# Ryo1011gd/ParticleMethod_FSI

Hardware: AMD Instinct MI355X
Metric: particle-steps/sec + achieved HBM GB/s, dam-break, 1/2/4/8 MI355X (higher is better)
Workload: dtype f64; 1 GPU; d1m: 3-D dam break (SURVEY 8d D1M, BASELINE configs[1]), 1397200 particles, ~1397200 per GPU; particles=1397200, dim=3, module=dam, parallelism=single

## Files before the change

include/mph_gpu.h:

```cpp
#ifndef MPH_GPU_H_INCLUDED
#define MPH_GPU_H_INCLUDED

#include <stddef.h>

#ifdef __cplusplus
extern "C" {
#endif

#define MPH_TYPE_COUNT 6
#define MPH_MAX_NEIGHBOR_COUNT 512
#define MPH_ABI_VERSION 6

typedef enum MphModule {
    MPH_MODULE_BAR = 0,
    MPH_MODULE_DAM = 1,
    MPH_MODULE_TUREK_HRON = 2,
    MPH_MODULE_ROLLING1 = 3,
    MPH_MODULE_HYDROELASTIC = 4,
    MPH_MODULE_NONE = 5
} MphModule;

typedef enum MphWallMotion {
    MPH_WALL_RIGID = 0,
    MPH_WALL_ROLLING = 1
// ... 229 lines not shown
    void* host_user;
    int n_glob;
    const int* ids;
    const double* cuts;
} MphSlabOptions;
int mph_create_slab(MphCtx** ctx, const MphConfig* cfg, int n, const int* property, const double* pos,
                    const double* pos0, const double* vel, int device, const MphSlabOptions* opt);
int mph_slab_window(const MphConfig* cfg, int rank, int nranks, int axis, const double* cuts, double* out2);
int mph_dist_selftest(int device);
int mph_dist_info(const MphCtx* ctx, int* out8);
int mph_dist_overlap(const MphCtx* ctx, double* out5);
int mph_list_stats(MphCtx* ctx, double* mean, int* max);
int mph_list_layout(MphCtx* ctx, long long out6[6]);
int mph_idle_wall_stats(MphCtx* ctx, long long out2[2]);
int mph_lean_step_stats(MphCtx* ctx, long long out2[2]);
int mph_neighbor_rows(MphCtx* ctx, int first, int count, int* counts, int* ids, long long ids_cap);
int mph_owned_count(const MphCtx* ctx);
int mph_owned_ids(MphCtx* ctx, int* out_ids);
int mph_slab_bounds(const MphConfig* cfg, int rank, int nranks, int axis, const double* cuts, double* out3);
int mph_slab_owner(const MphConfig* cfg, int nranks, int axis, const double* cuts, double c);

#ifdef __cplusplus
}
#endif
#endif
```

particlemethod_fsi_amd/csrc/mph_ctx.h:

```cpp
#pragma once

#include <hip/hip_runtime.h>

#include <map>
#include <string>
#include <thread>
#include <vector>

#include "mph_internal.h"
#include "mph_kernels.h"

struct MphDist;

struct MphCtx {
    int device = 0;
    int n = 0;
    int n_glob = 0;
    MphConfig cfg{};
    mph::HostDerived h{};
    mph::DevParams P{};
    mph::DevTables tables{};
    std::string err;
    std::thread out_thread;
    int out_rc = 0;
    double time = 0.0;
    bool stepped = false;
    hipStream_t stream = nullptr;
    hipGraphExec_t graph1 = nullptr, graph8 = nullptr;
    hipGraphExec_t graph1t = nullptr;
    bool batch_steps = false;
    int pending = 0;
    bool unchecked = false;
    void* hs_pin = nullptr;
    hipEvent_t ev_status = nullptr;
    bool phase_timing = false;
    std::vector<hipEvent_t> ev8, ev_vir;
    double phase_ms[3] = {0.0, 0.0, 0.0};
    std::vector<int> prop;
    std::vector<double> pos0;
    std::vector<int> gid;
    mph::StructureInit S;
    std::vector<int> sl_orig;
    std::vector<int> sl_s;
    int* order = nullptr;
// ... 119 lines not shown
    void join(hipStream_t waiting, hipStream_t from) override
    {
        hipEvent_t e = nullptr;
        (void)hipEventCreate(&e);
        (void)hipEventRecord(e, from);
        floors.push_back(e);
        pending[waiting] = (int)floors.size() - 1;
    }
    ~EventProfiler() override
    {
        for (auto& r : recs) { (void)hipEventDestroy(r.a); (void)hipEventDestroy(r.b); }
        for (auto e : floors) (void)hipEventDestroy(e);
    }
};

void enqueue_step(const Launch& L, bool last, hipEvent_t* ev = nullptr);

void ctx_set_global_error(const std::string& msg);
int ctx_create(MphCtx** out, const MphConfig* cfg, int n, const int* property, const double* pos,
               const double* pos0, const double* vel, int device, MphDist* dist, const int* ids = nullptr,
               int n_glob = 0);
template <typename T>
int fetch(MphCtx* c, const T* d, std::vector<T>& h, size_t count)
{
    h.resize(count);
    if (count) MPH_HIP_OK(c, hipMemcpyAsync(h.data(), d, sizeof(T) * count, hipMemcpyDeviceToHost, c->stream));
    return MPH_OK;
}

inline int glob_id(const MphCtx* c, int k) { return c->gid.empty() ? k : c->gid[k]; }

// ... 14 lines not shown
```

particlemethod_fsi_amd/csrc/mph_ctx.hip:

```cpp
#include <hip/hip_runtime.h>

#include <algorithm>
#include <cstring>
#include <string>

#include "mph_dist.h"
#include "mph_env.h"

using namespace mph;

namespace mph {

int ctx_fail(MphCtx* c, int code, const std::string& msg)
{
    if (c) c->err = msg;
    return code;
}

int ctx_hip_fail(MphCtx* c, hipError_t e, const char* what)
{
    return ctx_fail(c, e == hipErrorOutOfMemory ? MPH_ERR_DEVICE_OOM : MPH_ERR_HIP,
                    std::string(what) + ": " + hipGetErrorString(e));
}

// ... 42 lines not shown
    DevState hs;
    std::memcpy(&hs, c->hs_pin, kStateHead);
    return ctx_state_status(c, hs);
}

int ctx_status(MphCtx* c)
{
    MPH_CK(ctx_status_enqueue(c));
    MPH_HIP_OK(c, hipStreamSynchronize(c->stream));
    return ctx_status_landed(c);
}

int drop_graphs(MphCtx* c)
{
    MPH_HIP_OK(c, hipStreamSynchronize(c->stream));
    for (hipGraphExec_t* g : {&c->graph1, &c->graph1t, &c->graph8})
        if (*g) {
            MPH_HIP_OK(c, hipGraphExecDestroy(*g));
            *g = nullptr;
        }
    return MPH_OK;
}

int ctx_replay(MphCtx* c, int n)
{
    for (; n >= 8; n -= 8) MPH_HIP_OK(c, hipGraphLaunch(c->graph8, c->stream));
    for (; n > 1; --n) MPH_HIP_OK(c, hipGraphLaunch(c->graph1t ? c->graph1t : c->graph1, c->stream));
    if (n == 1) MPH_HIP_OK(c, hipGraphLaunch(c->graph1, c->stream));
    return MPH_OK;
}

void ctx_fill_launch(MphCtx* c)
{
    Launch& L = c->L;
    set_uniforms(c->P);
    if (env_int("MPH_LIST_FULL", 0) == 1) c->P.rlf = 3.0e38f;
    c->lazy_walls = !c->dist && env_int("MPH_LAZY_WALLS", 1) != 0;
    L.lean_ok = env_int("MPH_LEAN_STEPS", 1) != 0;
    L.lean_search = L.lean_ok && lean_search_ok(c->P);
    L.P = &c->P;
    L.stream = c->stream;
    L.xcd_bal_min = env_is("MPH_XCD_BAL_MIN", "") ? (1 << 20) : env_int("MPH_XCD_BAL_MIN", 1 << 20);
    L.S = &c->Sd;
}

}

extern "C" {

int mph_synchronize(MphCtx* c)
{
    if (!c) return MPH_ERR_ARG;
    MPH_CK(ctx_flush(c));
    MPH_HIP_OK(c, hipStreamSynchronize(c->stream));
// ... 11 lines not shown
    return MPH_OK;
}

void mph_destroy(MphCtx* c)
{
    if (!c) return;
    if (c->out_thread.joinable()) c->out_thread.join();
    (void)hipSetDevice(c->device);
    (void)ctx_flush(c);
    if (c->hs_pin) (void)hipHostFree(c->hs_pin);
    if (c->ev_status) (void)hipEventDestroy(c->ev_status);
    if (c->stream) (void)hipStreamSynchronize(c->stream);
    if (c->graph1) (void)hipGraphExecDestroy(c->graph1);
    if (c->graph1t) (void)hipGraphExecDestroy(c->graph1t);
    if (c->graph8) (void)hipGraphExecDestroy(c->graph8);
    for (auto* v : {&c->ev8, &c->ev_vir})
        for (hipEvent_t e : *v) (void)hipEventDestroy(e);
    if (c->dist) dist_free(c);
    for (void* p : c->allocs) (void)hipFree(p);
    if (c->stream) (void)hipStreamDestroy(c->stream);
    delete c;
}

}
```

particlemethod_fsi_amd/csrc/mph_device.h:

```cpp
#pragma once

#include <hip/hip_runtime.h>
#include <hip/hip_ext.h>

#include <climits>
#include <type_traits>

#include "mph_kernels.h"
#include "mph_params.h"

namespace mph {

__device__ __forceinline__ double mod_exact(double x, double w)
{
#pragma clang fp contract(off)
    return x - w * floor(x / w);
}

template <bool FAST>
__device__ __forceinline__ double image_exact(double d, double w, double hw, double w075)
{
#pragma clang fp contract(off)
    const double s = d + hw;
    double m;
// ... 113 lines not shown
{
    const int id = MAX ? INT_MIN : INT_MAX;
    auto op = [](int a, int b) { return MAX ? max(a, b) : min(a, b); };
    v = op(v, __builtin_amdgcn_update_dpp(id, v, 0x111, 0xf, 0xf, false));
    v = op(v, __builtin_amdgcn_update_dpp(id, v, 0x112, 0xf, 0xf, false));
    v = op(v, __builtin_amdgcn_update_dpp(id, v, 0x113, 0xf, 0xf, false));
    v = op(v, __builtin_amdgcn_update_dpp(id, v, 0x114, 0xf, 0xe, false));
    v = op(v, __builtin_amdgcn_update_dpp(id, v, 0x118, 0xf, 0xc, false));
    v = op(v, __builtin_amdgcn_update_dpp(id, v, 0x142, 0xa, 0xf, false));
    v = op(v, __builtin_amdgcn_update_dpp(id, v, 0x143, 0xc, 0xf, false));
    return __builtin_amdgcn_readlane(v, 63);
}

__device__ __forceinline__ int wave_min(int v) { return wave_reduce_dpp<false>(v); }
__device__ __forceinline__ int wave_max(int v) { return wave_reduce_dpp<true>(v); }

__device__ __forceinline__ void move_and_wrap(const DevParams& P, const DevState* st, Soa& B, int p,
                                              double& x, double& y, double& z)
{
#pragma clang fp contract(off)
    const int t = B.type[p];
    if (P.module == MPH_MODULE_TUREK_HRON && dev_is_fluid(t)) {
        const double ymin = 0.0, ymax = 0.41, umax = 1.0, h = ymax - ymin;
        if (x <= 0.01) {
            const double uy = y - ymin;
            B.vx[p] = (1.5 * 4.0 * umax / (h * h)) * uy * (h - uy);
            B.vy[p] = 0.0;
            B.vz[p] = 0.0;
        }
        if (x > 1.5 && st->time < 0.7) {
// ... 157 lines not shown
```

particlemethod_fsi_amd/csrc/mph_kernels.h:

```cpp
#pragma once

#include <hip/hip_runtime.h>

#include "mph_params.h"

namespace mph {

struct StructDev {
    int* orig = nullptr;
    int* slot_of = nullptr;
    int* bidx = nullptr;
    int n_own = 0;
    int n_inner = 0;
    int wo = 0, wi = 0;
    int* ocnt = nullptr;
    int* icnt = nullptr;
    int* eo_nb = nullptr;
    int* ei_nb = nullptr;
    double4* wx0 = nullptr;
    double* L = nullptr;
    double2* lame = nullptr;
    double* inv_rho = nullptr;
    int* clamp = nullptr;
    double4* x0 = nullptr;
// ... 41 lines not shown
    int width = 0;
    double probe_h = 0.0;
    long long* counters = nullptr;
    double* ring = nullptr;
    double* partial = nullptr;
    double* trk = nullptr;
    double* prb = nullptr;
    const int* track_sorted = nullptr;
    const int* track_map = nullptr;
    const double* probes = nullptr;
};

struct StepForm {
    bool lazy = false;
    bool lean_search = false, lean_pass_a = false;
};

struct Launch {
    const DevParams* P = nullptr;
    const DevTables* T = nullptr;
    DevState* st = nullptr;
    hipStream_t stream = nullptr;
    Profiler* prof = nullptr;
    Soa A, B;
    int* dst_of = nullptr;
    int *key = nullptr, *slot = nullptr, *tmp = nullptr, *cnt = nullptr, *start = nullptr, *bsum = nullptr;
    int *nbr = nullptr, *ncount = nullptr, *nbcount = nullptr;
    unsigned long long *lhdr = nullptr, *lgap = nullptr;
    int* wface = nullptr;
    VSrc vsrc;
    int xcd_bal_min = 1 << 20;
    unsigned char* cmap = nullptr;
    int cmap_bytes = 0;
    bool lean_ok = false, lean_search = false;
    StepForm form;
    double *pres = nullptr, *gx = nullptr, *gy = nullptr, *gz = nullptr, *pa = nullptr;
    double *dens_a = nullptr, *vstrain = nullptr, *divp = nullptr;
    double4 *fpart = nullptr;
    double4 *rec = nullptr;
    double4 *force = nullptr, *acc = nullptr;
    const StructDev* S = nullptr;
    const MonitorDev* mon = nullptr;
};

inline Launch trim_outputs(Launch L)
{
    L.dens_a = L.vstrain = L.divp = nullptr;
    if (!L.P->surface) L.gx = L.gy = L.gz = L.pa = nullptr;
    L.force = L.acc = nullptr;
    return L;
}

inline Launch step_launch(const Launch& L, bool last)
{
    Launch S = last ? L : trim_outputs(L);
    S.form.lazy = !last && L.cmap && !L.mon;
    S.form.lean_search = S.form.lazy && L.lean_ok && L.lean_search;
    S.form.lean_pass_a = S.form.lazy && L.lean_ok && !L.P->surface;
    return S;
}

struct SampleDev {
    double origin[3], spacing[3];
    int count[3];
    int tile[3];
    int tiles[3];
    int mask;
    double h;
};


int monitor_blocks(int n);
void launch_monitor(const Launch& L, const MonitorDev& M);
long long sample_tiling(SampleDev& G, int run_axis);
// ... 44 lines not shown
```

particlemethod_fsi_amd/csrc/mph_params.h:

```cpp
#pragma once
#include <cmath>

#include <cstddef>
#include <cstdint>

#include "../../include/mph_gpu.h"


namespace mph {

constexpr int kTypes = MPH_TYPE_COUNT;
constexpr int kMaxNeighbor = MPH_MAX_NEIGHBOR_COUNT;
constexpr int kTile = 64;
constexpr int kAlignRows = 128;
constexpr int kMaxJumps = 6;
#ifndef MPH_TILE_EXTRA
#define MPH_TILE_EXTRA kAlignRows
#endif
constexpr int kTileRows = kMaxNeighbor + MPH_TILE_EXTRA;
#ifndef MPH_TILE_PAD
#define MPH_TILE_PAD 1
#endif
constexpr int kTileStride = kTile * (kTileRows + MPH_TILE_PAD);
#if defined(__HIPCC__)
// ... 129 lines not shown
    int overflow;
    int pad0;
    int seam_occ[2];
    int seam_step;
    int seam_pad;
    int seg_work[kXcdSegs];
    int xcd_frac[9];
    int xcd_pad[3];
    unsigned long long lazy_steps;
    unsigned idle_waves[kXcdSegs];
    int seg_lwork[kXcdSegs];
    int seg_swork[kXcdSegs];
    int xcd_sfrac[9];
    int xcd_spad[3];
    unsigned long long lean_search_steps, lean_pass_a_steps;
};
constexpr size_t kStateHead = offsetof(DevState, seg_work);

#if defined(__HIPCC__)
#define MPH_HD __host__ __device__
#else
#define MPH_HD
#endif

MPH_HD inline int jump_count(unsigned long long hdr) { return (int)(hdr >> 56); }
MPH_HD inline int gap_begin(unsigned long long gap, int k) { return (int)((gap >> (8 * k)) & 0xff); }
MPH_HD inline int gap_end(unsigned long long hdr, int k) { return (int)((hdr >> (8 * k)) & 0xff); }

#ifndef MPH_PA_EQR
#define MPH_PA_EQR 1
// ... 74 lines not shown
```

particlemethod_fsi_amd/csrc/mph_passes.hip:

```cpp
#include <cstdio>
#include <cstdlib>
#include <type_traits>

#include "mph_list.h"

namespace mph {

__device__ __forceinline__ void own_velocity(const Soa& A, int i, double& vx, double& vy, double& vz)
{
    const double2 b = A.p6[3 * (size_t)i + 1], c = A.p6[3 * (size_t)i + 2];
    vx = b.y; vy = c.x; vz = c.y;
}


struct PassA {
    double da = 0.0, g0 = 0.0, g1 = 0.0, g2 = 0.0, vs = 0.0, dv = 0.0;
    double s0 = 0.0, s1 = 0.0, s2 = 0.0, v0 = 0.0, v1 = 0.0, v2 = 0.0;
};

template <bool FORCE, bool EQR = false, bool LEAN = false>
__device__ __forceinline__ void pass_a_term(const DevParams& P, const double* s_ratio, const double* s_mu, int ti,
                                            int tj, bool solid, double q0, double q1, double q2, double r2,
                                            double dvx, double dvy, double dvz, PassA& o)
{
// ... 313 lines not shown
        for (int u = 0; u < U; ++u) {
            const unsigned off = ok[u] ? (unsigned)jj[u] * 16u : kGatherOob;
            const double2 a = buf_ld16(recr, off), b = buf_ld16(recr, off == kGatherOob ? off : off + ps16);
            X[u] = a.x; Y[u] = a.y; Z[u] = b.x; PJ[u] = b.y;
        }
#pragma unroll
        for (int u = 0; u < U; ++u) {
            asm volatile("" ::"v"(X[u]), "v"(Y[u]), "v"(Z[u]), "v"(PJ[u]));
            if (!ok[u]) continue;
            pass_b_term<FAST, SURF, DIM>(P, s_ratio, gx, gy, gz, pa, jj[u], TT[u], X[u], Y[u], Z[u], PJ[u], ti,
                                         solid, xi, yi, zi, gxi, gyi, gzi, pai, ai, dscale, cpv, f0, f1, f2);
        }
    }
}

template <bool SURF, int DIM>
#ifndef MPH_PB_WPE
#define MPH_PB_WPE 0
#endif
#if MPH_PB_WPE
#define MPH_PB_ATTR __attribute__((amdgpu_waves_per_eu(MPH_PB_WPE)))
#else
#define MPH_PB_ATTR
#endif
__global__ __launch_bounds__(MPH_LB) MPH_PB_ATTR void k_pass_b(DevParams P, const DevTables* __restrict__ T, Soa A,
                                                const double4* __restrict__ rec,
                                                const double4* __restrict__ fpart,
                                                const double* __restrict__ gx,
                                                const double* __restrict__ gy,
                                                const double* __restrict__ gz,
                                                const double* __restrict__ pa,
                                                const int* __restrict__ nbr,
                                                const int* __restrict__ ncount,
                                                const unsigned long long* __restrict__ lhdr,
                                                const unsigned long long* __restrict__ lgap,
                                                double4* __restrict__ force, double4* __restrict__ acc,
                                                Soa B, int phase, int* __restrict__ wface, StructHook H,
                                                const DevState* __restrict__ st)
{
    const int n = dev_n(P);
    const int lb = list_block(st, n);
    if (lb < 0) return;
    __shared__ double s_ratio[kTypes * kTypes];
    if (SURF) {
        if (threadIdx.x < kTypes * kTypes) s_ratio[threadIdx.x] = T->ratio[threadIdx.x];
        __syncthreads();
    }
    const int i = lb * blockDim.x + threadIdx.x;
    const int ii = i < n ? i : n - 1;
    const double xi = A.x[ii], yi = A.y[ii], zi = A.z[ii];
    bool live = i < n;
    if (phase) {
        const int f = wface[__builtin_amdgcn_readfirstlane(i >> 6)];
        if (phase == 1 ? f != 0 : f == 0) return;
    }
    if (wave_all_ghosts(P, A, live, ii)) {
        if (live) B.id[i] = A.id[i];
        return;
    }
    if (live && P.slab_axis >= 0 && A.id[ii] < 0) {
        B.id[i] = A.id[i];
        live = false;
    }
    const bool fast = wave_search_interior(P, st, live, xi, yi, zi);
    if (!live) return;
    const int ti = A.type[ii];
    const bool solid = dev_is_struct(ti);
    const double4 fp = fpart[ii];
    double f0 = fp.x, f1 = fp.y, f2 = fp.z;
    double gxi = 0.0, gyi = 0.0, gzi = 0.0, pai = 0.0, ai = 0.0;
    if (SURF) {
        gxi = gx[ii]; gyi = gy[ii]; gzi = gz[ii]; pai = pa[ii];
        ai = T->cofa[ti] * P.cofk * P.cofk;
    }
    const int end = !force && dev_is_wall(ti) ? 0 : (ncount[i] < kTileRows ? ncount[i] : kTileRows);
    const unsigned long long hdr = wave_hdr(lhdr, i);
    const bool plain = (hdr >> 56) == 0;
    const RowMask M = row_mask(hdr, lgap, i, end);
    const NbrList NL = nbr_list(nbr, i);
    if (fast)
        pass_b_loop<true, SURF, DIM>(P, s_ratio, rec, gx, gy, gz, pa, NL, plain, M, end, ti, solid, xi, yi, zi, gxi,
                                     gyi, gzi, pai, ai, f0, f1, f2);
    else
        pass_b_loop<false, SURF, DIM>(P, s_ratio, rec, gx, gy, gz, pa, NL, plain, M, end, ti, solid, xi, yi, zi, gxi,
                                      gyi, gzi, pai, ai, f0, f1, f2);
    double vxi, vyi, vzi;
    own_velocity(A, i, vxi, vyi, vzi);
    double vo0 = vxi, vo1 = vyi, vo2 = vzi;
    double xo0 = xi, xo1 = yi, xo2 = zi;
    double4 ao = make_double4(0.0, 0.0, 0.0, 0.0);
    if (dev_is_fluid(ti) || solid) {
        const double m = T->mass[ti], im = T->inv_mass[ti];
        f0 += m * P.gravity[0];
        f1 += m * P.gravity[1];
        f2 += m * P.gravity[2];
        vo0 += f0 * im * P.dt;
        vo1 += f1 * im * P.dt;
        vo2 += f2 * im * P.dt;
        if (!solid) {
            ao = make_double4(f0 * im, f1 * im, f2 * im, 0.0);
            xo0 += vo0 * P.dt;
            xo1 += vo1 * P.dt;
            xo2 += vo2 * P.dt;
        }
    }
    if (force) {
        force[i] = make_double4(f0, f1, f2, 0.0);
        acc[i] = ao;
    }
    B.x[i] = xo0;
    B.y[i] = xo1;
    B.z[i] = xo2;
    B.vx[i] = vo0;
    B.vy[i] = vo1;
    B.vz[i] = vo2;
    B.type[i] = ti;
    B.id[i] = A.id[i];
    const int id = A.id[i];
    if (solid && H.slot_of && id >= 0) {
// ... 117 lines not shown
        h.su = L.S->u;
        h.sx0 = L.S->x0;
        h.bidx = L.S->bidx;
    }
    return h;
}

void launch_pass_b(const Launch& L, int phase)
{
    const DevParams& P = *L.P;
    if (P.n == 0) return;
    if (P.surface && !(L.gx && L.gy && L.gz && L.pa)) {
        std::fprintf(stderr, "mph: launch_pass_b with surface tension needs GravityCenter/PressureA\n");
        std::abort();
    }
    auto go = [&](auto SURF) {
        by_dim(P.dim, [&](auto D) {
            launch(L.prof, phase == 2 ? "pass_b_face" : "pass_b", L.stream,
                   k_pass_b<decltype(SURF)::value, decltype(D)::value>,
                   dim3(list_grid(P.n, L.form.lazy && P.n >= L.xcd_bal_min)), dim3(MPH_LB), P, L.T, L.A,
                   L.rec, L.fpart, L.gx, L.gy, L.gz, L.pa, L.nbr, L.ncount, L.lhdr, L.lgap, L.force, L.acc, L.B, phase,
                   L.wface, struct_hook(L), L.st);
        });
    };
    if (P.surface) go(std::true_type{});
    else go(std::false_type{});
}

void launch_virial(const Launch& L, const Soa& X, double* vir, double* vpres)
{
    const DevParams& P = *L.P;
    if (P.n == 0) return;
    by_dim(P.dim, [&](auto D) {
        launch(L.prof, "virial", L.stream, k_virial<decltype(D)::value>, dim3(blocks(P.n, 256)), dim3(256), P, L.T,
               L.A, X, L.pres, L.pa, L.gx, L.gy, L.gz, L.nbr, L.ncount, L.lhdr, L.lgap, vir, vpres);
    });
}

}
```

particlemethod_fsi_amd/csrc/mph_profile.hip:

```cpp
#include <hip/hip_runtime.h>

#include <algorithm>
#include <cstddef>
#include <cstdio>
#include <map>
#include <string>
#include <vector>

#include "mph_dist.h"
#include "mph_rows.h"

using namespace mph;

extern "C" {

int mph_profile_steps(MphCtx* c, int nsteps, double* avg_ms, int* launches, char* names32)
{
    if (nsteps <= 0 || !avg_ms || !launches || !names32) return MPH_ERR_ARG;
    MPH_CK(ctx_enter(c));
    EventProfiler prof;
    if (c->dist) {
        MPH_CK(dist_step(c, nsteps, &prof));
    } else {
        Launch L = c->L;
        L.prof = &prof;
        for (int k = 0; k < nsteps; ++k) enqueue_step(L, k == nsteps - 1);
        MPH_HIP_OK(c, hipGetLastError());
        MPH_HIP_OK(c, hipStreamSynchronize(c->stream));
        ctx_stepped(c, nsteps, true);
    }
    std::vector<std::string> order;
    std::map<std::string, std::pair<double, int>> acc;
    std::vector<std::pair<float, float>> span;
    for (auto& r : prof.recs) {
        float ms = 0.0f, t0 = 0.0f;
        MPH_HIP_OK(c, hipEventElapsedTime(&ms, r.a, r.b));
        MPH_HIP_OK(c, hipEventElapsedTime(&t0, prof.recs[0].a, r.a));
        if (r.floor >= 0) {
            float tf = 0.0f;
            MPH_HIP_OK(c, hipEventElapsedTime(&tf, prof.recs[0].a, prof.floors[r.floor]));
            if (tf > t0) {
// ... 166 lines not shown
int mph_lean_step_stats(MphCtx* c, long long out[2])
{
    if (!out) return MPH_ERR_ARG;
    MPH_CK(ctx_enter(c));
    MPH_HIP_OK(c, hipStreamSynchronize(c->stream));
    unsigned long long steps[2] = {0, 0};
    static_assert(offsetof(DevState, lean_pass_a_steps) == offsetof(DevState, lean_search_steps) + sizeof(steps[0]),
                  "the two counters are read in one copy");
    MPH_HIP_OK(c, hipMemcpy(steps, reinterpret_cast<const char*>(c->L.st) + offsetof(DevState, lean_search_steps),
                            sizeof(steps), hipMemcpyDeviceToHost));
    out[0] = (long long)steps[0];
    out[1] = (long long)steps[1];
    return MPH_OK;
}

int mph_neighbor_rows(MphCtx* c, int first, int count, int* counts, int* ids, long long ids_cap)
{
    if (!c || first < 0 || count < 0 || !counts || (!ids && ids_cap > 0)) return MPH_ERR_ARG;
    MPH_CK(ctx_flush(c));
    if (c->dist) return ctx_fail(c, MPH_ERR_UNSUPPORTED, "mph_neighbor_rows: single contexts only");
    if ((long long)first + count > c->n) return ctx_fail(c, MPH_ERR_ARG, "mph_neighbor_rows: range past the particle count");
    if (!count) return 0;
    MPH_HIP_OK(c, hipSetDevice(c->device));
    const int n = c->n;
    if (c->P.rlf < 3.0e38f)
        return ctx_fail(c, MPH_ERR_UNSUPPORTED, "mph_neighbor_rows: the lists keep only the pairs within the passes' "
                                            "radius (create the context with MPH_LIST_FULL=1 for the reference's lists)");
    std::vector<int> id(n), nv(n);
    MPH_HIP_OK(c, hipMemcpy(id.data(), c->L.A.id, sizeof(int) * n, hipMemcpyDeviceToHost));
    MPH_HIP_OK(c, hipMemcpy(nv.data(), c->L.nbcount, sizeof(int) * n, hipMemcpyDeviceToHost));
// ... 45 lines not shown
```

particlemethod_fsi_amd/csrc/mph_sort.hip:

```cpp
#include "mph_device.h"

namespace mph {


__device__ __forceinline__ int seam_bits(const DevParams& P, double x, double y, double z)
{
    const double v[3] = {x, y, z};
    int b = 0;
#pragma unroll
    for (int k = 0; k < 3; ++k) {
        if (k == 2 && P.dim == 2) break;
        if ((P.seam_always >> k) & 1) continue;
        b |= (v[k] < P.inner_lo[k] ? 1 : 0) << (2 * k);
        b |= (v[k] > P.inner_hi[k] ? 2 : 0) << (2 * k);
    }
    return b;
}

constexpr int kScanThreads = 256;
#ifndef MPH_SCAN_ITEMS
#define MPH_SCAN_ITEMS 16
#endif
constexpr int kScanItems = MPH_SCAN_ITEMS;
constexpr int kScanBlock = kScanThreads * kScanItems;
__host__ __device__ inline int bsum_stride(int ncell) { return ncell / kScanBlock + 2; }
static_assert(kScanBlock == 4096, "mph_create.hip sizes the bsum buffer for 4096-cell blocks");

template <int T>
__device__ __forceinline__ void xcd_split_block(int* seg, int* fr)
{
    constexpr int R = kXcdSegs / T;
    static_assert(kXcdSegs % T == 0, "whole runs per thread");
// ... 206 lines not shown
        }
    } else {
#pragma unroll
        for (int k = 0; k < kScanItems; ++k)
            if (base + k < ncell) {
                start[base + k] = o[k];
                if (v[k] != 0) cnt[base + k] = 0;
            }
    }
    if (blockIdx.x == 0 && threadIdx.x == 0) start[ncell] = n_dev ? *n_dev : n;
}

__global__ __launch_bounds__(256) void k_place(DevParams P, DevState* __restrict__ st,
                                               const int* __restrict__ key, const int* __restrict__ slot,
                                               const int* __restrict__ start, int* __restrict__ tmp,
                                               int mode)
{
    const int p = blockIdx.x * blockDim.x + threadIdx.x;
    if (blockIdx.x == 0 && threadIdx.x == 0) {
        st->seam_occ[(st->seam_step + 1) & 1] = 0;
        st->seam_step += 1;
        if (mode) {
#pragma clang fp contract(off)
            for (int t = 4; t < 6; ++t)
                for (int d = 0; d < 3; ++d) st->wall_c[t][d] += st->wall_vel[t][d] * P.dt;
            st->time += P.dt;
        }
    }
    const int n = dev_n(P);
    if (p >= n) return;
    const int d = start[key[p]] + slot[p];
    if ((unsigned)d >= (unsigned)n) {
        atomicOr(&st->overflow, 64);
        return;
    }
    tmp[d] = p;
}

__global__ __launch_bounds__(256) void k_rank_scatter(DevParams P, const int* __restrict__ key,
                                                      const int* __restrict__ start,
                                                      const int* __restrict__ tmp, Soa C, Soa A,
                                                      int* __restrict__ rank_of, int* __restrict__ dst_of,
// ... 40 lines not shown
    const int nb = blocks(ncell, kScanBlock);
    const int top = nb <= kScanFusedTop;
    launch(prof, "scan_reduce", stream, k_scan_reduce, dim3(nb), dim3(kScanThreads), cnt, ncell, bsum);
    if (!top) launch(prof, "scan_top", stream, k_scan_top, dim3(1), dim3(1024), bsum, nb);
    launch(prof, "scan_down", stream, k_scan_down, dim3(nb), dim3(kScanThreads), cnt, ncell, bsum, start, total,
           n_dev, top);
}

void launch_sort(const Launch& L, int mode)
{
    const DevParams& P = *L.P;
    const int n = P.n;
    if (n == 0) return;
    const int split = n >= L.xcd_bal_min ? (L.form.lazy ? 2 : 1) : 0;
    const dim3 g(blocks(n, 256)), b(256);
    launch(L.prof, "prep", L.stream, k_prep, g, b, P, L.st, L.B, L.key, L.slot, L.cnt, mode, L.vsrc,
           L.form.lazy ? L.cmap : nullptr);
    launch_scan(L.cnt, P.ncell, L.bsum, L.start, n, P.n_dev, L.stream, L.prof);
    launch(L.prof, "place", L.stream, k_place, g, b, P, L.st, L.key, L.slot, L.start, L.tmp, mode);
    launch(L.prof, "rank_scatter", L.stream, k_rank_scatter, g, b, P, L.key, L.start, L.tmp, L.B, L.A,
           nullptr , L.dst_of, mode,
           L.vsrc, L.st, split);
}

}
```

particlemethod_fsi_amd/csrc/mph_step.hip:

```cpp
#include <hip/hip_runtime.h>

#include <vector>

#include "mph_dist.h"

using namespace mph;

namespace mph {

void enqueue_step(const Launch& L, bool last, hipEvent_t* ev)
{
    if (ev) (void)hipEventRecord(ev[0], L.stream);
    const Launch S = step_launch(L, last);
    launch_sort(S, 1);
    if (ev) {
        launch_neighbors(S);
        (void)hipEventRecord(ev[1], L.stream);
        launch_pass_a(S);
    } else {
        launch_search_pass_a(S);
    }
    launch_pass_b(S);
    launch_structure(L, last);
    if (ev) (void)hipEventRecord(ev[2], L.stream);
    if (L.mon) launch_monitor(L, *L.mon);
}

static int capture(MphCtx* c, int steps, hipGraphExec_t* out, bool store_last = true)
{
    return ctx_capture(c, steps, out, [&](int k) {
        enqueue_step(c->L, store_last && k == steps - 1);
        return MPH_OK;
    });
}

static int capture_graphs(MphCtx* c)
{
    if (!c->graph1) MPH_CK(capture(c, 1, &c->graph1));
    if (!c->graph1t) MPH_CK(capture(c, 1, &c->graph1t, false));
    if (!c->graph8) MPH_CK(capture(c, 8, &c->graph8));
    return MPH_OK;
}

static int accumulate_phases(MphCtx* c, const std::vector<hipEvent_t>& ev, int steps)
{
    MPH_HIP_OK(c, hipEventSynchronize(ev[3 * (size_t)steps - 1]));
    for (size_t k = 0; k + 2 < 3 * (size_t)steps; k += 3) {
        float a = 0.0f, b = 0.0f;
        MPH_HIP_OK(c, hipEventElapsedTime(&a, ev[k], ev[k + 1]));
        MPH_HIP_OK(c, hipEventElapsedTime(&b, ev[k + 1], ev[k + 2]));
        c->phase_ms[0] += a;
        c->phase_ms[1] += b;
    }
    return MPH_OK;
}
// ... 44 lines not shown
    return MPH_OK;
}

int mph_step(MphCtx* c, int nsteps)
{
    if (!c || nsteps < 0) return MPH_ERR_ARG;
    MPH_HIP_OK(c, hipSetDevice(c->device));
    if (c->dist) return dist_step(c, nsteps);
    if (nsteps == 0 || c->n == 0) {
        ctx_advance_time(c, nsteps);
        return MPH_OK;
    }
    if (c->batch_steps && !c->phase_timing) return step_batched(c, nsteps);
    MPH_CK(ctx_flush(c));
    if (c->phase_timing) {
        for (int left = nsteps; left > 0;) {
            const int b = left >= 8 ? 8 : 1;
            for (int k = 0; k < b; ++k) enqueue_step(c->L, k == b - 1, c->ev8.data() + 3 * k);
            MPH_HIP_OK(c, hipGetLastError());
            MPH_CK(accumulate_phases(c, c->ev8, b));
            left -= b;
        }
    } else {
        MPH_CK(capture_graphs(c));
        MPH_CK(ctx_replay(c, nsteps));
    }
    ctx_stepped(c, nsteps, true);
    return ctx_status(c);
}

int mph_phase_timing(MphCtx* c, int on)
{
    if (!c) return MPH_ERR_ARG;
    MPH_CK(ctx_flush(c));
    if (c->dist) return on ? ctx_fail(c, MPH_ERR_ARG, "phase timing is not available in slab mode") : MPH_OK;
    MPH_HIP_OK(c, hipSetDevice(c->device));
    const bool want = on != 0;
// ... 21 lines not shown
```

particlemethod_fsi_amd/solver.py:

```python
from __future__ import annotations

import ctypes
import os
import subprocess

import numpy as np

from . import mphio

PKG_DIR = os.path.dirname(os.path.abspath(__file__))
LIB_DIR = os.path.join(PKG_DIR, "lib")
LIB_PATH = os.environ.get("MPH_GPU_LIB") or os.path.join(LIB_DIR, "libmph_gpu.so")
CSRC_DIR = os.path.join(PKG_DIR, "csrc")

FIELDS = {
    "Position": (0, 3, np.float64), "InitialPosition": (1, 3, np.float64),
    "Velocity": (2, 3, np.float64), "Force": (3, 3, np.float64),
    "Acceleration": (4, 3, np.float64), "GravityCenter": (5, 3, np.float64),
    "PressureP": (6, 1, np.float64), "PressureA": (7, 1, np.float64),
    "DensityA": (8, 1, np.float64), "VolStrainP": (9, 1, np.float64),
    "DivergenceP": (10, 1, np.float64), "Mass": (11, 1, np.float64), "Kappa": (12, 1, np.float64),
    "Lambda": (13, 1, np.float64), "Mu": (14, 1, np.float64),
    "NeighborCount": (15, 1, np.int32), "InitialStructureNeighborCount": (16, 1, np.int32),
    "Property": (17, 1, np.int32), "DeformGradient": (18, 9, np.float64),
# ... 11 lines not shown
EXPORTED_SYMBOLS = [
    "mph_config_default", "mph_read_data_file", "mph_read_grid_header", "mph_read_grid_particles",
    "mph_write_prof_arrays", "mph_write_vtk_arrays", "mph_create", "mph_step", "mph_synchronize",
    "mph_get", "mph_set", "mph_particle_count", "mph_time", "mph_get_scalars", "mph_write_prof",
    "mph_write_vtk", "mph_last_error", "mph_destroy", "mph_profile_steps", "mph_profile_graphs", "mph_neighbor_stats",
    "mph_dist_unique_id", "mph_create_dist", "mph_owned_count", "mph_derive_scalars",
    "mph_structure_init", "mph_create_dist_host", "mph_owned_ids", "mph_slab_bounds",
    "mph_slab_owner", "mph_dist_selftest", "mph_compute_virial",
    "mph_config_sizeof", "mph_write_vtk_async", "mph_output_wait", "mph_write_grid_binary",
    "mph_write_vtu_arrays", "mph_write_vtu", "mph_velocity_profile_arrays",
    "mph_set_initial_velocity_profile", "mph_dist_info", "mph_create_slab", "mph_slab_window",
    "mph_list_stats", "mph_abi_version", "mph_phase_timing", "mph_phase_times",
    "mph_set_step_batching", "mph_neighbor_rows", "mph_dist_overlap", "mph_list_layout",
    "mph_monitor_configure", "mph_monitor_sample_doubles", "mph_monitor_read",
    "mph_sample_grid", "mph_sample_grid_timed", "mph_write_vti_arrays", "mph_idle_wall_stats",
    "mph_lean_step_stats",
]

ABI_VERSION = 6

HOST_EXCHANGE_FN = ctypes.CFUNCTYPE(ctypes.c_int, ctypes.c_void_p, ctypes.c_void_p, ctypes.c_size_t,
                                    ctypes.c_void_p, ctypes.c_size_t, ctypes.c_void_p, ctypes.c_size_t,
                                    ctypes.c_void_p, ctypes.c_size_t)


class MphSlabOptions(ctypes.Structure):
    _fields_ = [("rank", ctypes.c_int), ("nranks", ctypes.c_int), ("axis", ctypes.c_int),
                ("unique_id128", ctypes.c_char_p), ("host_fn", HOST_EXCHANGE_FN),
                ("host_user", ctypes.c_void_p), ("n_glob", ctypes.c_int), ("ids", ctypes.c_void_p),
                ("cuts", ctypes.c_void_p)]

# ... 122 lines not shown
        "mph_slab_window": (ip, [cfgp, ip, ip, ip, vp, vp]),
        "mph_phase_timing": (ip, [vp, ip]),
        "mph_phase_times": (ip, [vp, vp]),
        "mph_set_step_batching": (ip, [vp, ip]),
        "mph_neighbor_rows": (ip, [vp, ip, ip, vp, vp, ctypes.c_longlong]),
        "mph_dist_overlap": (ip, [vp, vp]),
        "mph_list_layout": (ip, [vp, vp]),
        "mph_monitor_configure": (ip, [vp, ctypes.POINTER(MphMonitorConfig)]),
        "mph_monitor_sample_doubles": (ip, [vp]),
        "mph_monitor_read": (ctypes.c_longlong, [vp, vp, ctypes.c_longlong, ctypes.POINTER(ctypes.c_longlong)]),
        "mph_sample_grid": (ip, [vp, ctypes.POINTER(MphSampleGrid), vp]),
        "mph_sample_grid_timed": (ip, [vp, ctypes.POINTER(MphSampleGrid), vp, ctypes.POINTER(ctypes.c_double), vp]),
        "mph_write_vti_arrays": (ip, [ctypes.c_char_p, ctypes.POINTER(MphSampleGrid), vp]),
        "mph_idle_wall_stats": (ip, [vp, vp]),
        "mph_lean_step_stats": (ip, [vp, vp]),
    }
    optional = {"mph_phase_timing", "mph_phase_times", "mph_set_step_batching", "mph_neighbor_rows",
                "mph_dist_overlap", "mph_profile_graphs", "mph_list_stats", "mph_list_layout",
                "mph_monitor_configure", "mph_monitor_sample_doubles", "mph_monitor_read",
                "mph_sample_grid", "mph_sample_grid_timed", "mph_write_vti_arrays", "mph_idle_wall_stats",
                "mph_lean_step_stats"}
    for name, (res, args) in sig.items():
        if name in optional and not hasattr(L, name):
            continue
        f = getattr(L, name)
        f.restype = res
        f.argtypes = args
    accept = {ABI_VERSION} | {int(v) for v in os.environ.get("MPH_ABI_ACCEPT", "").split(",") if v.strip()}
    if L.mph_abi_version() not in accept:
        raise ImportError("%s has C ABI version %d, these bindings expect %d (rebuild the library)"
                          % (LIB_PATH, L.mph_abi_version(), ABI_VERSION))
    if L.mph_config_sizeof() != ctypes.sizeof(mphio.MphConfig):
        raise ImportError("MphConfig layout mismatch between %s and mphio.MphConfig" % LIB_PATH)
    _lib = L
    return L

# ... 328 lines not shown
        keys = ["waves", "waves_jumped", "jumps", "max_jumps", "gap_rows", "max_rows"]
        return {k: int(v) for k, v in zip(keys, a)}

    def idle_wall_stats(self) -> dict:
        a = np.zeros(2, np.int64)
        if hasattr(self._L, "mph_idle_wall_stats"):
            _check(self._L.mph_idle_wall_stats(self._h, a.ctypes.data), self._h)
        return {"idle_wave_steps": int(a[0]), "lazy_steps": int(a[1])}

    def lean_step_stats(self) -> dict:
        a = np.zeros(2, np.int64)
        if hasattr(self._L, "mph_lean_step_stats"):
            _check(self._L.mph_lean_step_stats(self._h, a.ctypes.data), self._h)
        return {"search_steps": int(a[0]), "pass_a_steps": int(a[1])}

    def neighbor_rows(self, first: int = 0, count: int | None = None):
        if count is None:
            count = self.n - first
        counts = np.zeros(count, np.int32)
        cap = max(1, count * 128)
        while True:
            ids = np.zeros(cap, np.int32)
            r = self._L.mph_neighbor_rows(self._h, int(first), int(count), counts.ctypes.data, ids.ctypes.data, cap)
            need = int(np.minimum(counts, 512).sum()) if r == -1 else 0
            if r == -1 and need > cap:
                cap = need
                continue
            _check(r, self._h)
            break
        offsets = np.concatenate([[0], np.cumsum(np.minimum(counts, 512))]).astype(np.int64)
# ... 41 lines not shown
```

Baseline: 1.526 billion particle-steps/s.

## Fold next-step sort key/slot computation into pass_b and add lean 8-step graph

Pass_b gains a KEYS variant. It moves and wraps each particle, computes its cell key, does a wave-aggregated atomic count into the cell histogram, writes the slot and coarse map, and ORs in the seam bits. The next step's sort can then skip the separate k_prep kernel launch and its extra read/write of particle state. A graph8t capture without storing the last step is also added, and replay now prefers lean 8-step batches. The cost is more register pressure and branching in pass_b, a whole-wave early exit instead of a per-thread one, and more graph memory.

```diff
diff --git a/include/mph_gpu.h b/include/mph_gpu.h
--- a/include/mph_gpu.h
+++ b/include/mph_gpu.h
@@ -267,6 +267,7 @@
 int mph_list_layout(MphCtx* ctx, long long out6[6]);
 int mph_idle_wall_stats(MphCtx* ctx, long long out2[2]);
 int mph_lean_step_stats(MphCtx* ctx, long long out2[2]);
+int mph_key_fold_stats(MphCtx* ctx, long long out2[2]);
 int mph_neighbor_rows(MphCtx* ctx, int first, int count, int* counts, int* ids, long long ids_cap);
 int mph_owned_count(const MphCtx* ctx);
 int mph_owned_ids(MphCtx* ctx, int* out_ids);
diff --git a/particlemethod_fsi_amd/csrc/mph_ctx.h b/particlemethod_fsi_amd/csrc/mph_ctx.h
--- a/particlemethod_fsi_amd/csrc/mph_ctx.h
+++ b/particlemethod_fsi_amd/csrc/mph_ctx.h
@@ -28,6 +28,8 @@
     hipStream_t stream = nullptr;
     hipGraphExec_t graph1 = nullptr, graph8 = nullptr;
     hipGraphExec_t graph1t = nullptr;
+    hipGraphExec_t graph8t = nullptr;
+    bool lean_calls = false;
     bool batch_steps = false;
     int pending = 0;
     bool unchecked = false;
@@ -177,7 +179,8 @@
     }
 };
 
-void enqueue_step(const Launch& L, bool last, hipEvent_t* ev = nullptr);
+void enqueue_step(const Launch& L, bool last, hipEvent_t* ev = nullptr, int k = 0, int steps = 1,
+                  bool next_last = true);
 
 void ctx_set_global_error(const std::string& msg);
 int ctx_create(MphCtx** out, const MphConfig* cfg, int n, const int* property, const double* pos,
diff --git a/particlemethod_fsi_amd/csrc/mph_ctx.hip b/particlemethod_fsi_amd/csrc/mph_ctx.hip
--- a/particlemethod_fsi_amd/csrc/mph_ctx.hip
+++ b/particlemethod_fsi_amd/csrc/mph_ctx.hip
@@ -80,7 +80,7 @@
 int drop_graphs(MphCtx* c)
 {
     MPH_HIP_OK(c, hipStreamSynchronize(c->stream));
-    for (hipGraphExec_t* g : {&c->graph1, &c->graph1t, &c->graph8})
+    for (hipGraphExec_t* g : {&c->graph1, &c->graph1t, &c->graph8, &c->graph8t})
         if (*g) {
             MPH_HIP_OK(c, hipGraphExecDestroy(*g));
             *g = nullptr;
@@ -90,9 +90,11 @@
 
 int ctx_replay(MphCtx* c, int n)
 {
-    for (; n >= 8; n -= 8) MPH_HIP_OK(c, hipGraphLaunch(c->graph8, c->stream));
-    for (; n > 1; --n) MPH_HIP_OK(c, hipGraphLaunch(c->graph1t ? c->graph1t : c->graph1, c->stream));
-    if (n == 1) MPH_HIP_OK(c, hipGraphLaunch(c->graph1, c->stream));
+    const ReplayPlan p = replay_plan(n, c->graph8t != nullptr, c->graph1t != nullptr);
+    for (int k = 0; k < p.batch8t; ++k) MPH_HIP_OK(c, hipGraphLaunch(c->graph8t, c->stream));
+    for (int k = 0; k < p.batch8; ++k) MPH_HIP_OK(c, hipGraphLaunch(c->graph8, c->stream));
+    for (int k = 0; k < p.single1t; ++k) MPH_HIP_OK(c, hipGraphLaunch(c->graph1t, c->stream));
+    for (int k = 0; k < p.single1; ++k) MPH_HIP_OK(c, hipGraphLaunch(c->graph1, c->stream));
     return MPH_OK;
 }
 
@@ -104,6 +106,8 @@
     c->lazy_walls = !c->dist && env_int("MPH_LAZY_WALLS", 1) != 0;
     L.lean_ok = env_int("MPH_LEAN_STEPS", 1) != 0;
     L.lean_search = L.lean_ok && lean_search_ok(c->P);
+    c->lean_calls = !c->dist && env_int("MPH_LEAN_CALLS", 1) != 0;
+    L.key_fold = !c->dist && env_int("MPH_KEY_FOLD", 1) != 0;
     L.P = &c->P;
     L.stream = c->stream;
     L.xcd_bal_min = env_is("MPH_XCD_BAL_MIN", "") ? (1 << 20) : env_int("MPH_XCD_BAL_MIN", 1 << 20);
@@ -145,6 +149,7 @@
     if (c->graph1) (void)hipGraphExecDestroy(c->graph1);
     if (c->graph1t) (void)hipGraphExecDestroy(c->graph1t);
     if (c->graph8) (void)hipGraphExecDestroy(c->graph8);
+    if (c->graph8t) (void)hipGraphExecDestroy(c->graph8t);
     for (auto* v : {&c->ev8, &c->ev_vir})
         for (hipEvent_t e : *v) (void)hipEventDestroy(e);
     if (c->dist) dist_free(c);
diff --git a/particlemethod_fsi_amd/csrc/mph_device.h b/particlemethod_fsi_amd/csrc/mph_device.h
--- a/particlemethod_fsi_amd/csrc/mph_device.h
+++ b/particlemethod_fsi_amd/csrc/mph_device.h
@@ -151,6 +151,20 @@
 
 __device__ __forceinline__ int wave_min(int v) { return wave_reduce_dpp<false>(v); }
 __device__ __forceinline__ int wave_max(int v) { return wave_reduce_dpp<true>(v); }
+
+__device__ __forceinline__ int seam_bits(const DevParams& P, double x, double y, double z)
+{
+    const double v[3] = {x, y, z};
+    int b = 0;
+#pragma unroll
+    for (int k = 0; k < 3; ++k) {
+        if (k == 2 && P.dim == 2) break;
+        if ((P.seam_always >> k) & 1) continue;
+        b |= (v[k] < P.inner_lo[k] ? 1 : 0) << (2 * k);
+        b |= (v[k] > P.inner_hi[k] ? 2 : 0) << (2 * k);
+    }
+    return b;
+}
 
 __device__ __forceinline__ void move_and_wrap(const DevParams& P, const DevState* st, Soa& B, int p,
                                               double& x, double& y, double& z)
diff --git a/particlemethod_fsi_amd/csrc/mph_kernels.h b/particlemethod_fsi_amd/csrc/mph_kernels.h
--- a/particlemethod_fsi_amd/csrc/mph_kernels.h
+++ b/particlemethod_fsi_amd/csrc/mph_kernels.h
@@ -79,6 +79,7 @@
 struct StepForm {
     bool lazy = false;
     bool lean_search = false, lean_pass_a = false;
+    bool keys_done = false, keys_next = false;
 };
 
 struct Launch {
@@ -98,6 +99,8 @@
     unsigned char* cmap = nullptr;
     int cmap_bytes = 0;
     bool lean_ok = false, lean_search = false;
+    bool key_fold = false;
+    unsigned char* cmap_next = nullptr;
     StepForm form;
     double *pres = nullptr, *gx = nullptr, *gy = nullptr, *gz = nullptr, *pa = nullptr;
     double *dens_a = nullptr, *vstrain = nullptr, *divp = nullptr;
@@ -123,6 +126,34 @@
     S.form.lean_search = S.form.lazy && L.lean_ok && L.lean_search;
     S.form.lean_pass_a = S.form.lazy && L.lean_ok && !L.P->surface;
     return S;
+}
+
+inline bool key_fold_ok(const Launch& L)
+{
+    return L.key_fold && L.P->n_struct == 0 && !L.mon && !L.vsrc.idx;
+}
+inline Launch step_keys(Launch S, const Launch& L, int k, int steps, bool next_last)
+{
+    const bool ok = key_fold_ok(L);
+    S.form.keys_done = ok && k > 0;
+    S.form.keys_next = ok && k + 1 < steps;
+    S.cmap_next = S.form.keys_next && step_launch(L, next_last).form.lazy ? L.cmap : nullptr;
+    return S;
+}
+
+struct ReplayPlan {
+    int batch8t = 0, batch8 = 0, single1t = 0, single1 = 0;
+};
+inline ReplayPlan replay_plan(int n, bool lean8, bool lean1)
+{
+    ReplayPlan p;
+    if (n <= 0) return p;
+    const int whole = n / 8, rest = n % 8;
+    p.batch8t = lean8 && whole >= 2 ? whole - 1 : 0;
+    p.batch8 = whole - p.batch8t;
+    p.single1t = lean1 && rest > 1 ? rest - 1 : 0;
+    p.single1 = rest - p.single1t;
+    return p;
 }
 
 struct SampleDev {
diff --git a/particlemethod_fsi_amd/csrc/mph_params.h b/particlemethod_fsi_amd/csrc/mph_params.h
--- a/particlemethod_fsi_amd/csrc/mph_params.h
+++ b/particlemethod_fsi_amd/csrc/mph_params.h
@@ -167,6 +167,7 @@
     int xcd_sfrac[9];
     int xcd_spad[3];
     unsigned long long lean_search_steps, lean_pass_a_steps;
+    unsigned long long key_fold_steps, prep_steps;
 };
 constexpr size_t kStateHead = offsetof(DevState, seg_work);
 
diff --git a/particlemethod_fsi_amd/csrc/mph_passes.hip b/particlemethod_fsi_amd/csrc/mph_passes.hip
--- a/particlemethod_fsi_amd/csrc/mph_passes.hip
+++ b/particlemethod_fsi_amd/csrc/mph_passes.hip
@@ -351,7 +351,12 @@
     }
 }
 
-template <bool SURF, int DIM>
+struct KeyOut {
+    int *key, *slot, *cnt;
+    unsigned char* cmap;
+};
+
+template <bool SURF, int DIM, bool KEYS = false>
 #ifndef MPH_PB_WPE
 #define MPH_PB_WPE 0
 #endif
@@ -373,11 +378,12 @@
                                                 const unsigned long long* __restrict__ lgap,
                                                 double4* __restrict__ force, double4* __restrict__ acc,
                                                 Soa B, int phase, int* __restrict__ wface, StructHook H,
-                                                const DevState* __restrict__ st)
+                                                const DevState* __restrict__ st, KeyOut K)
 {
     const int n = dev_n(P);
     const int lb = list_block(st, n);
     if (lb < 0) return;
+    if (KEYS && lb == 0 && threadIdx.x == 0) const_cast<DevState*>(st)->key_fold_steps += 1;
     __shared__ double s_ratio[kTypes * kTypes];
     if (SURF) {
         if (threadIdx.x < kTypes * kTypes) s_ratio[threadIdx.x] = T->ratio[threadIdx.x];
@@ -400,7 +406,9 @@
         live = false;
     }
     const bool fast = wave_search_interior(P, st, live, xi, yi, zi);
-    if (!live) return;
+    if (!KEYS && !live) return;
+    if (KEYS && !__any(live)) return;
+    const int ir = KEYS ? ii : i;
     const int ti = A.type[ii];
     const bool solid = dev_is_struct(ti);
     const double4 fp = fpart[ii];
@@ -410,11 +418,11 @@
         gxi = gx[ii]; gyi = gy[ii]; gzi = gz[ii]; pai = pa[ii];
         ai = T->cofa[ti] * P.cofk * P.cofk;
     }
-    const int end = !force && dev_is_wall(ti) ? 0 : (ncount[i] < kTileRows ? ncount[i] : kTileRows);
-    const unsigned long long hdr = wave_hdr(lhdr, i);
+    const int end = !force && dev_is_wall(ti) ? 0 : (ncount[ir] < kTileRows ? ncount[ir] : kTileRows);
+    const unsigned long long hdr = wave_hdr(lhdr, ir);
     const bool plain = (hdr >> 56) == 0;
-    const RowMask M = row_mask(hdr, lgap, i, end);
-    const NbrList NL = nbr_list(nbr, i);
+    const RowMask M = row_mask(hdr, lgap, ir, end);
+    const NbrList NL = nbr_list(nbr, ir);
     if (fast)
         pass_b_loop<true, SURF, DIM>(P, s_ratio, rec, gx, gy, gz, pa, NL, plain, M, end, ti, solid, xi, yi, zi, gxi,
                                      gyi, gzi, pai, ai, f0, f1, f2);
@@ -422,7 +430,7 @@
         pass_b_loop<false, SURF, DIM>(P, s_ratio, rec, gx, gy, gz, pa, NL, plain, M, end, ti, solid, xi, yi, zi, gxi,
                                       gyi, gzi, pai, ai, f0, f1, f2);
     double vxi, vyi, vzi;
-    own_velocity(A, i, vxi, vyi, vzi);
+    own_velocity(A, ir, vxi, vyi, vzi);
     double vo0 = vxi, vo1 = vyi, vo2 = vzi;
     double xo0 = xi, xo1 = yi, xo2 = zi;
     double4 ao = make_double4(0.0, 0.0, 0.0, 0.0);
@@ -440,6 +448,50 @@
             xo1 += vo1 * P.dt;
             xo2 += vo2 * P.dt;
         }
+    }
+    if (KEYS) {
+        const int lane = threadIdx.x & 63;
+        int k = -1 - lane;
+        int occ = 0;
+        if (live) {
+            B.vx[i] = vo0;
+            B.vy[i] = vo1;
+            B.vz[i] = vo2;
+            B.type[i] = ti;
+            B.id[i] = A.id[i];
+            double x = xo0, y = xo1, z = xo2;
+            move_and_wrap(P, st, B, i, x, y, z);
+            if (!isfinite(x + y + z)) atomicOr(const_cast<int*>(&st->overflow), 4);
+            const int cx = cell_axis(x, P.corg[0], P.dw[0], P.ginv[0], P.gc[0]);
+            const int cy = cell_axis(y, P.corg[1], P.dw[1], P.ginv[1], P.gc[1]);
+            const int cz = P.dim == 3 ? cell_axis(z, P.corg[2], P.dw[2], P.ginv[2], P.gc[2]) : 0;
+            k = cell_index(P, cx, cy, cz);
+            K.key[i] = k;
+            if (K.cmap && !dev_is_wall(ti))
+                K.cmap[coarse_index(P, cx >> kCoarseShift, cy >> kCoarseShift, cz >> kCoarseShift)] = 1;
+            occ = seam_bits(P, x, y, z);
+        }
+        const int kprev = __shfl_up(k, 1, 64);
+        const bool head = lane == 0 || kprev != k;
+        const unsigned long long heads = __ballot(head);
+        const unsigned long long upto = lane == 63 ? ~0ull : ((2ull << lane) - 1ull);
+        const int hl = 63 - __clzll(heads & upto);
+        const unsigned long long above = heads & ~upto;
+        const int next = above ? __ffsll((long long)above) - 1 : 64;
+        int base = 0;
+        if (live && head) base = atomicAdd(&K.cnt[k], next - lane);
+        base = __shfl(base, hl, 64);
+        if (live) K.slot[i] = base + (lane - hl);
+        if (__ballot(occ != 0)) {
+#pragma unroll
+            for (int o = 32; o > 0; o >>= 1) occ |= __shfl_xor(occ, o, 64);
+            if (lane == 0) {
+                int* w = const_cast<int*>(&st->seam_occ[st->seam_step & 1]);
+                const int cur = __hip_atomic_load(w, __ATOMIC_RELAXED, __HIP_MEMORY_SCOPE_AGENT);
+                if (occ & ~cur) atomicOr(w, occ);
+            }
+        }
+        return;
     }
     if (force) {
         force[i] = make_double4(f0, f1, f2, 0.0);
@@ -587,17 +639,22 @@
         std::fprintf(stderr, "mph: launch_pass_b with surface tension needs GravityCenter/PressureA\n");
         std::abort();
     }
-    auto go = [&](auto SURF) {
+    const bool keys = L.form.keys_next;
+    if (keys && (L.force || P.n_struct > 0 || phase || P.slab_axis >= 0 || P.n_dev)) {
+        std::fprintf(stderr, "mph: launch_pass_b: the key fold on a step that cannot take it\n");
+        std::abort();
+    }
+    auto go = [&](auto SURF, auto KEYS) {
         by_dim(P.dim, [&](auto D) {
             launch(L.prof, phase == 2 ? "pass_b_face" : "pass_b", L.stream,
-                   k_pass_b<decltype(SURF)::value, decltype(D)::value>,
+                   k_pass_b<decltype(SURF)::value, decltype(D)::value, decltype(KEYS)::value>,
                    dim3(list_grid(P.n, L.form.lazy && P.n >= L.xcd_bal_min)), dim3(MPH_LB), P, L.T, L.A,
                    L.rec, L.fpart, L.gx, L.gy, L.gz, L.pa, L.nbr, L.ncount, L.lhdr, L.lgap, L.force, L.acc, L.B, phase,
-                   L.wface, struct_hook(L), L.st);
+                   L.wface, struct_hook(L), L.st, keys ? KeyOut{L.key, L.slot, L.cnt, L.cmap_next} : KeyOut{});
         });
     };
-    if (P.surface) go(std::true_type{});
-    else go(std::false_type{});
+    if (P.surface) keys ? go(std::true_type{}, std::true_type{}) : go(std::true_type{}, std::false_type{});
+    else keys ? go(std::false_type{}, std::true_type{}) : go(std::false_type{}, std::false_type{});
 }
 
 void launch_virial(const Launch& L, const Soa& X, double* vir, double* vpres)
diff --git a/particlemethod_fsi_amd/csrc/mph_profile.hip b/particlemethod_fsi_amd/csrc/mph_profile.hip
--- a/particlemethod_fsi_amd/csrc/mph_profile.hip
+++ b/particlemethod_fsi_amd/csrc/mph_profile.hip
@@ -24,7 +24,7 @@
     } else {
         Launch L = c->L;
         L.prof = &prof;
-        for (int k = 0; k < nsteps; ++k) enqueue_step(L, k == nsteps - 1);
+        for (int k = 0; k < nsteps; ++k) enqueue_step(L, k == nsteps - 1, nullptr, k, nsteps, k + 1 == nsteps - 1);
         MPH_HIP_OK(c, hipGetLastError());
         MPH_HIP_OK(c, hipStreamSynchronize(c->stream));
         ctx_stepped(c, nsteps, true);
@@ -221,6 +221,21 @@
     return MPH_OK;
 }
 
+int mph_key_fold_stats(MphCtx* c, long long out[2])
+{
+    if (!out) return MPH_ERR_ARG;
+    MPH_CK(ctx_enter(c));
+    MPH_HIP_OK(c, hipStreamSynchronize(c->stream));
+    unsigned long long steps[2] = {0, 0};
+    static_assert(offsetof(DevState, prep_steps) == offsetof(DevState, key_fold_steps) + sizeof(steps[0]),
+                  "the two counters are read in one copy");
+    MPH_HIP_OK(c, hipMemcpy(steps, reinterpret_cast<const char*>(c->L.st) + offsetof(DevState, key_fold_steps),
+                            sizeof(steps), hipMemcpyDeviceToHost));
+    out[0] = (long long)steps[0];
+    out[1] = (long long)steps[1];
+    return MPH_OK;
+}
+
 int mph_neighbor_rows(MphCtx* c, int first, int count, int* counts, int* ids, long long ids_cap)
 {
     if (!c || first < 0 || count < 0 || !counts || (!ids && ids_cap > 0)) return MPH_ERR_ARG;
diff --git a/particlemethod_fsi_amd/csrc/mph_sort.hip b/particlemethod_fsi_amd/csrc/mph_sort.hip
--- a/particlemethod_fsi_amd/csrc/mph_sort.hip
+++ b/particlemethod_fsi_amd/csrc/mph_sort.hip
@@ -2,20 +2,6 @@
 
 namespace mph {
 
-
-__device__ __forceinline__ int seam_bits(const DevParams& P, double x, double y, double z)
-{
-    const double v[3] = {x, y, z};
-    int b = 0;
-#pragma unroll
-    for (int k = 0; k < 3; ++k) {
-        if (k == 2 && P.dim == 2) break;
-        if ((P.seam_always >> k) & 1) continue;
-        b |= (v[k] < P.inner_lo[k] ? 1 : 0) << (2 * k);
-        b |= (v[k] > P.inner_hi[k] ? 2 : 0) << (2 * k);
-    }
-    return b;
-}
 
 constexpr int kScanThreads = 256;
 #ifndef MPH_SCAN_ITEMS
@@ -252,7 +238,7 @@
 __global__ __launch_bounds__(256) void k_place(DevParams P, DevState* __restrict__ st,
                                                const int* __restrict__ key, const int* __restrict__ slot,
                                                const int* __restrict__ start, int* __restrict__ tmp,
-                                               int mode)
+                                               int mode, int prep)
 {
     const int p = blockIdx.x * blockDim.x + threadIdx.x;
     if (blockIdx.x == 0 && threadIdx.x == 0) {
@@ -264,6 +250,7 @@
                 for (int d = 0; d < 3; ++d) st->wall_c[t][d] += st->wall_vel[t][d] * P.dt;
             st->time += P.dt;
         }
+        if (prep) st->prep_steps += 1;
     }
     const int n = dev_n(P);
     if (p >= n) return;
@@ -334,10 +321,13 @@
     if (n == 0) return;
     const int split = n >= L.xcd_bal_min ? (L.form.lazy ? 2 : 1) : 0;
     const dim3 g(blocks(n, 256)), b(256);
-    launch(L.prof, "prep", L.stream, k_prep, g, b, P, L.st, L.B, L.key, L.slot, L.cnt, mode, L.vsrc,
-           L.form.lazy ? L.cmap : nullptr);
+    const bool prep = !(mode == 1 && L.form.keys_done);
+    if (prep)
+        launch(L.prof, "prep", L.stream, k_prep, g, b, P, L.st, L.B, L.key, L.slot, L.cnt, mode, L.vsrc,
+               L.form.lazy ? L.cmap : nullptr);
     launch_scan(L.cnt, P.ncell, L.bsum, L.start, n, P.n_dev, L.stream, L.prof);
-    launch(L.prof, "place", L.stream, k_place, g, b, P, L.st, L.key, L.slot, L.start, L.tmp, mode);
+    launch(L.prof, "place", L.stream, k_place, g, b, P, L.st, L.key, L.slot, L.start, L.tmp, mode,
+           (int)(prep && mode == 1));
     launch(L.prof, "rank_scatter", L.stream, k_rank_scatter, g, b, P, L.key, L.start, L.tmp, L.B, L.A,
            nullptr , L.dst_of, mode,
            L.vsrc, L.st, split);
diff --git a/particlemethod_fsi_amd/csrc/mph_step.hip b/particlemethod_fsi_amd/csrc/mph_step.hip
--- a/particlemethod_fsi_amd/csrc/mph_step.hip
+++ b/particlemethod_fsi_amd/csrc/mph_step.hip
@@ -8,10 +8,10 @@
 
 namespace mph {
 
-void enqueue_step(const Launch& L, bool last, hipEvent_t* ev)
+void enqueue_step(const Launch& L, bool last, hipEvent_t* ev, int k, int steps, bool next_last)
 {
     if (ev) (void)hipEventRecord(ev[0], L.stream);
-    const Launch S = step_launch(L, last);
+    const Launch S = step_keys(step_launch(L, last), L, k, steps, next_last);
     launch_sort(S, 1);
     if (ev) {
         launch_neighbors(S);
@@ -29,7 +29,7 @@
 static int capture(MphCtx* c, int steps, hipGraphExec_t* out, bool store_last = true)
 {
     return ctx_capture(c, steps, out, [&](int k) {
-        enqueue_step(c->L, store_last && k == steps - 1);
+        enqueue_step(c->L, store_last && k == steps - 1, nullptr, k, steps, store_last && k + 1 == steps - 1);
         return MPH_OK;
     });
 }
@@ -39,6 +39,7 @@
     if (!c->graph1) MPH_CK(capture(c, 1, &c->graph1));
     if (!c->graph1t) MPH_CK(capture(c, 1, &c->graph1t, false));
     if (!c->graph8) MPH_CK(capture(c, 8, &c->graph8));
+    if (c->lean_calls && !c->graph8t) MPH_CK(capture(c, 8, &c->graph8t, false));
     return MPH_OK;
 }
 
@@ -113,13 +114,16 @@
     if (c->batch_steps && !c->phase_timing) return step_batched(c, nsteps);
     MPH_CK(ctx_flush(c));
     if (c->phase_timing) {
-        for (int left = nsteps; left > 0;) {
-            const int b = left >= 8 ? 8 : 1;
-            for (int k = 0; k < b; ++k) enqueue_step(c->L, k == b - 1, c->ev8.data() + 3 * k);
-            MPH_HIP_OK(c, hipGetLastError());
-            MPH_CK(accumulate_phases(c, c->ev8, b));
-            left -= b;
-        }
+        const ReplayPlan p = replay_plan(nsteps, c->lean_calls, true);
+        const int batches[4][3] = {{p.batch8t, 8, 0}, {p.batch8, 8, 1}, {p.single1t, 1, 0}, {p.single1, 1, 1}};
+        for (const auto& [count, b, store_last] : batches)
+            for (int r = 0; r < count; ++r) {
+                for (int k = 0; k < b; ++k)
+                    enqueue_step(c->L, store_last && k == b - 1, c->ev8.data() + 3 * k, k, b,
+                                 store_last && k + 1 == b - 1);
+                MPH_HIP_OK(c, hipGetLastError());
+                MPH_CK(accumulate_phases(c, c->ev8, b));
+            }
     } else {
         MPH_CK(capture_graphs(c));
         MPH_CK(ctx_replay(c, nsteps));
diff --git a/particlemethod_fsi_amd/solver.py b/particlemethod_fsi_amd/solver.py
--- a/particlemethod_fsi_amd/solver.py
+++ b/particlemethod_fsi_amd/solver.py
@@ -49,7 +49,7 @@
     "mph_set_step_batching", "mph_neighbor_rows", "mph_dist_overlap", "mph_list_layout",
     "mph_monitor_configure", "mph_monitor_sample_doubles", "mph_monitor_read",
     "mph_sample_grid", "mph_sample_grid_timed", "mph_write_vti_arrays", "mph_idle_wall_stats",
-    "mph_lean_step_stats",
+    "mph_lean_step_stats", "mph_key_fold_stats",
 ]
 
 ABI_VERSION = 6
@@ -202,12 +202,13 @@
         "mph_write_vti_arrays": (ip, [ctypes.c_char_p, ctypes.POINTER(MphSampleGrid), vp]),
         "mph_idle_wall_stats": (ip, [vp, vp]),
         "mph_lean_step_stats": (ip, [vp, vp]),
+        "mph_key_fold_stats": (ip, [vp, vp]),
     }
     optional = {"mph_phase_timing", "mph_phase_times", "mph_set_step_batching", "mph_neighbor_rows",
                 "mph_dist_overlap", "mph_profile_graphs", "mph_list_stats", "mph_list_layout",
                 "mph_monitor_configure", "mph_monitor_sample_doubles", "mph_monitor_read",
                 "mph_sample_grid", "mph_sample_grid_timed", "mph_write_vti_arrays", "mph_idle_wall_stats",
-                "mph_lean_step_stats"}
+                "mph_lean_step_stats", "mph_key_fold_stats"}
     for name, (res, args) in sig.items():
         if name in optional and not hasattr(L, name):
             continue
@@ -566,6 +567,12 @@
             _check(self._L.mph_lean_step_stats(self._h, a.ctypes.data), self._h)
         return {"search_steps": int(a[0]), "pass_a_steps": int(a[1])}
 
+    def key_fold_stats(self) -> dict:
+        a = np.zeros(2, dtype=np.int64)
+        if hasattr(self._L, "mph_key_fold_stats"):
+            _check(self._L.mph_key_fold_stats(self._h, a.ctypes.data), self._h)
+        return {"folded_steps": int(a[0]), "prep_launches": int(a[1])}
+
     def neighbor_rows(self, first: int = 0, count: int | None = None):
         if count is None:
             count = self.n - first
```

New measurement: 1.594 billion particle-steps/s, median of 6. 4.4% higher.
